# mobilinkd/m17-cxx-demod

Measured on AMD Instinct MI355X. Metric: Msamples/s demodulated (48 kSPS 4-FSK in -> decoded frames), higher is better.
Workload: dtype f32

## Files before the change

m17-cxx-demod_amd/csrc/m17_fir_skew_body.inc:

```
    __shared__ __attribute__((aligned(16))) float win[FS_LDS_FLOATS];
    const int tid = threadIdx.x;
    typedef int v4i __attribute__((ext_vector_type(4)));
    constexpr int NCH = (FS_WIN + 7) / 8;
    constexpr int CPT = (NCH + FS_THREADS - 1) / FS_THREADS;
    constexpr bool F32 = std::is_same<XT, float>::value;
    constexpr int FS_LAST = FS_WIN - 16 * FS_THREADS;
    static_assert(FS_LAST > 0 && FS_LAST <= FS_THREADS && CPT == 3, "the float form's split of the window");
    v4i pre[F32 ? 4 : CPT];
    int pre_last = 0;
    int m = 0;
    auto fetch = [&](uint32_t item) {
        const uint32_t c = item / tiles, tile = item - c * tiles;
        const XT* xr = x + (size_t)c * xpitch + XPRE;
        const int64_t w0 = (int64_t)tile * FS_TILE - FS_WOFF;
#pragma unroll
        for (int q = 0; q < CPT; ++q) {
            const int k = tid + q * FS_THREADS;
            const int64_t t = w0 + 8 * k;
            v4i v = {0, 0, 0, 0};
            if constexpr (F32) {
                if (q < 2) {
                    v4i v2 = {0, 0, 0, 0};
                    if (t + 8 <= (int64_t)T) {
                        v = *reinterpret_cast<const v4i*>(xr + t);
                        v2 = *reinterpret_cast<const v4i*>(xr + t + 4);
                    } else {
                        uint32_t w[8];
#pragma unroll
                        for (int h = 0; h < 8; ++h) w[h] = t + h < (int64_t)T ? __float_as_uint(xr[t + h]) : 0u;
                        v = v4i{(int)w[0], (int)w[1], (int)w[2], (int)w[3]};
                        v2 = v4i{(int)w[4], (int)w[5], (int)w[6], (int)w[7]};
                    }
                    pre[2 * q] = v; pre[2 * q + 1] = v2;
                } else {
                    const int64_t tl = w0 + 16 * FS_THREADS + tid;
                    pre_last = (tid < FS_LAST && tl < (int64_t)T) ? (int)__float_as_uint(xr[tl]) : 0;
                }
            } else {
            if (k < NCH) {
                if (t + 8 <= (int64_t)T) v = *reinterpret_cast<const v4i*>(xr + t);
                else {
                    uint32_t w[4] = {0u, 0u, 0u, 0u};
#pragma unroll 1
                    for (int h = 0; h < 8; ++h)
                        if (t + h < (int64_t)T) w[h >> 1] |= (uint32_t)(uint16_t)xr[t + h] << (16 * (h & 1));
                    v = v4i{(int)w[0], (int)w[1], (int)w[2], (int)w[3]};
                }
            }
            pre[q] = v;
            }
        }
    };
    auto stage = [&] {
#pragma unroll
        for (int q = 0; q < CPT; ++q) {
            const int k = tid + q * FS_THREADS;
            int sm = INVERT ? (int)0x80000000u : 0;
            if constexpr (F32 && MIXED) sm = m & (int)0x80000000u;
            if constexpr (F32) if (q == 2) {
                const int j = 16 * FS_THREADS + tid;
                if (tid < FS_LAST) win[FS_PADF + j + 2 * (j >> 4)] = __int_as_float(pre_last ^ sm);
                continue;
            }
            if (k < NCH) {
                float* dst = win + FS_PADF + 8 * k + 2 * (k >> 1);
                if constexpr (F32) {
#pragma unroll
                    for (int h = 0; h < 4; ++h) {
                        const v4i r = pre[2 * q + (h >> 1)];
                        const int a = ((h & 1) ? r[2] : r[0]) ^ sm, b = ((h & 1) ? r[3] : r[1]) ^ sm;
                        *reinterpret_cast<v2f*>(dst + 2 * h) = v2f{__int_as_float(a), __int_as_float(b)};
                    }
                } else
#pragma unroll
                for (int h = 0; h < 4; ++h) {
                    int w = pre[q][h];
// ... 80 lines not shown
```

m17-cxx-demod_amd/csrc/m17_frontend_kernels.hpp:

```cpp
#pragma once

#include "m17_common.hpp"

#include <type_traits>

namespace m17 {

typedef float v2f __attribute__((ext_vector_type(2)));

template <bool INVERT>
__device__ __forceinline__ v2f dcd_scale2(int a, int b)
{
    if (INVERT) { a = (int)(int16_t)(-a); b = (int)(int16_t)(-b); }
    const v2f rcp = {1.0f / 41067.0f, 1.0f / 41067.0f};
    const v2f k = {41067.0f, 41067.0f};
    const v2f fs = {(float)a, (float)b};
    const v2f q = fs * rcp;
    const v2f r = __builtin_elementwise_fma(-q, k, fs);
    return __builtin_elementwise_fma(r, rcp, q);
}

__device__ __forceinline__ int pol_mask(const uint32_t* __restrict__ pol, uint32_t c, uint32_t flip) { return -(int)((pol[c] ^ flip) & 1u); }
__device__ __forceinline__ int pol_word(int w, int m)
{
// ... 109 lines not shown
    }
}

#endif

template <int E, int N, typename F>
__device__ __forceinline__ void static_for(F&& f)
{
    if constexpr (E < N) {
        f(std::integral_constant<int, E>{});
        static_for<E + 1, N>(f);
    }
}

constexpr int FS_R = 16;
constexpr int FS_THREADS = 256;
constexpr int FS_TILE = FS_R * FS_THREADS;
constexpr int FS_WOFF = 152;
constexpr int FS_WIN = FS_TILE + FS_WOFF;
constexpr int FS_PADF = 18;
constexpr int FS_LDS_FLOATS = FS_PADF + ((FS_WIN + 15) / 16) * 18;
constexpr int FS_STEPS = 150, FS_BODY = 32, FS_ENTRY = 10, FS_NBODY = 5;
static_assert(FS_BODY - FS_ENTRY + (FS_NBODY - 1) * FS_BODY == FS_STEPS, "step count");
constexpr int FS_TAB = 64;

constexpr int fs_off(int e) { return e + 2 * ((e - (e < 0 ? 15 : 0)) / 16); }

inline void fs_build_tap_table(float* tab )
{
    auto T2 = [](int s) { return (s >= 1 && s <= 149) ? rrc_tap(s - 1) : 0.0f; };
    for (int bi = 0; bi < FS_NBODY; ++bi)
        for (int k = 0; k < 32; ++k) {
            const int s = 32 * (bi - 1) + (FS_BODY - FS_ENTRY) + k;
            tab[bi * FS_TAB + k] = T2(s);
            tab[bi * FS_TAB + 32 + k] = T2(s + 1);
        }
}

template <int HALF>
__device__ __forceinline__ v2f fs_tap_pair_times(v2f taps, v2f wpair)
{
    v2f r;
    if constexpr (HALF) asm("v_pk_mul_f32 %0, %1, %2 op_sel:[0,1] op_sel_hi:[1,1]" : "=v"(r) : "s"(taps), "v"(wpair));
    else asm("v_pk_mul_f32 %0, %1, %2 op_sel:[0,0] op_sel_hi:[1,0]" : "=v"(r) : "s"(taps), "v"(wpair));
    return r;
}

template <bool INVERT>
__global__ __launch_bounds__(FS_THREADS, 4) void fir_rrc150_skew_kernel(const int16_t* __restrict__ x, size_t xpitch, float* __restrict__ y, size_t ypitch,
                                                                       uint32_t T, const float* __restrict__ tab, uint32_t tiles, uint32_t items,
                                                                       const uint32_t* __restrict__ first_needed)
{
    constexpr bool MIXED = false;
    const uint32_t* pol = nullptr; const uint32_t flip = 0u;
    typedef int16_t XT;
#include "m17_fir_skew_body.inc"
}
__global__ __launch_bounds__(FS_THREADS, 4) void fir_rrc150_skew_mixed_kernel(const int16_t* __restrict__ x, size_t xpitch, float* __restrict__ y, size_t ypitch,
                                                                             uint32_t T, const float* __restrict__ tab, uint32_t tiles, uint32_t items,
                                                                             const uint32_t* __restrict__ first_needed, const uint32_t* __restrict__ pol, uint32_t flip)
{
    constexpr bool INVERT = false, MIXED = true;
    typedef int16_t XT;
#include "m17_fir_skew_body.inc"
}
template <bool INVERT>
__global__ __launch_bounds__(FS_THREADS, 4) void fir_rrc150_skew_f32_kernel(const float* __restrict__ x, size_t xpitch, float* __restrict__ y, size_t ypitch,
                                                                           uint32_t T, const float* __restrict__ tab, uint32_t tiles, uint32_t items,
                                                                           const uint32_t* __restrict__ first_needed)
{
    constexpr bool MIXED = false;
    const uint32_t* pol = nullptr; const uint32_t flip = 0u;
    typedef float XT;
#include "m17_fir_skew_body.inc"
}
__global__ __launch_bounds__(FS_THREADS, 4) void fir_rrc150_skew_mixed_f32_kernel(const float* __restrict__ x, size_t xpitch, float* __restrict__ y, size_t ypitch,
                                                                                 uint32_t T, const float* __restrict__ tab, uint32_t tiles, uint32_t items,
                                                                                 const uint32_t* __restrict__ first_needed, const uint32_t* __restrict__ pol, uint32_t flip)
{
    constexpr bool INVERT = false, MIXED = true;
    typedef float XT;
#include "m17_fir_skew_body.inc"
}

__global__ __launch_bounds__(256) void correlate_kernel(const float* __restrict__ y, size_t ypitch, float* __restrict__ corr,
                                                        uint32_t C, uint32_t T, uint32_t t0, uint32_t Ttot)
{
    const uint32_t c = blockIdx.y;
    const uint32_t t = t0 + blockIdx.x * blockDim.x + threadIdx.x;
    if (t >= t0 + T) return;
    const float* yr = y + (size_t)c * ypitch + YPRE;
// ... 461 lines not shown
```

m17-cxx-demod_amd/csrc/m17_gate_kernel.hpp:

```cpp
#pragma once

#include "m17_common.hpp"
#include "m17_decode_device.hpp"
#include "m17_frontend_kernels.hpp"
#include "m17_state.hpp"

namespace m17 {

struct GateExport {
    int32_t init;
    uint32_t on, trig, count;
    int32_t run_pos;
    float h0, h1, h2;
    float level;
    uint32_t seg;
    int32_t end_in_run, end_t;
};

struct GateParams {
    const int16_t* x;
    size_t xpitch;
    const float* y;
    size_t ypitch;
    float* h;
// ... 3 lines not shown
    const GateExport* chain_in;
    GateExport* chain_out;
    const uint32_t* only;
    const Boundary* bnd;
    float* final_h;
    const float* taps;
    uint32_t C, T;
    uint64_t pos0;
    uint64_t tick_row0;
    uint32_t flags;
    uint32_t nblk;
    EvParams ev;
    const uint32_t* pol;
    const float* hist_f;
    const float* bnd_hist_f;
};

constexpr int GT_LPC = 4;
constexpr int GT_CPW = 64 / GT_LPC;
constexpr int GT_ROW = TICK + 4;
constexpr int GT_F4 = TICK / 4 / GT_LPC;
constexpr int GT_LDS_FLOATS = GT_CPW * GT_ROW + GT_CPW * 148 + 298;

template <typename XT>
__device__ __forceinline__ void limit_track_pass(const GateParams& P, bool state_only, uint32_t c, bool valid, bool from_chain, const Boundary* bnd_base,
                                                 float* lds_base)
{
    constexpr uint32_t t0 = 0;
    const uint32_t segT = P.T;
    const size_t fh_off = 0;
    const Boundary* bnd = bnd_base ? bnd_base + c : nullptr;
    const uint64_t pos0 = P.pos0 + t0;
    float (&yl)[GT_CPW][GT_ROW] = *reinterpret_cast<float (*)[GT_CPW][GT_ROW]>(lds_base);
    float (&hl)[GT_CPW][GT_ROW] = yl;
    float (&pl)[GT_CPW][148] = *reinterpret_cast<float (*)[GT_CPW][148]>(lds_base + GT_CPW * GT_ROW);
    float (&pw)[298] = *reinterpret_cast<float (*)[298]>(lds_base + GT_CPW * GT_ROW + GT_CPW * 148);
    const int lane = threadIdx.x;
    const int g = lane % GT_CPW, r = lane / GT_CPW;
    const bool invert = ((P.flags ^ (P.pol ? P.pol[c] : 0u)) & 1u) != 0u;
    const bool store = !state_only;
    const SeqState* gs = P.state + c;
    const float* yr = P.y + (size_t)c * P.ypitch + YPRE + t0;
    float* hr = P.h + (size_t)c * P.ypitch + YPRE + t0;
    const float* tab = P.dcd_table + (size_t)c * P.ticks_cap * 12;

    int32_t init, run_pos, end_t = 0;
    uint32_t on, trig, count, seg;
    float h0, h1, h2, level;
    bool end_in_run = false;
    if (from_chain) {
        const GateExport e = P.chain_in[c];
// ... 8 lines not shown
        on = gs->hot.dcd_on; trig = gs->hot.dcd_trig; count = gs->hot.count;
        run_pos = gs->hot.run_pos;
        h0 = gs->hot.h0; h1 = gs->hot.h1; h2 = gs->hot.h2;
        level = gs->cold.dcd_level;
        seg = gs->cold.seg_start_tick;
    }
    if (!valid) { init = 0; on = 0; trig = 0; count = 0; run_pos = 148; h0 = h1 = h2 = 0.f; level = 0.f; seg = 0; end_in_run = false; end_t = 0; }
    if (!from_chain && r == 0 && valid && store) { hr[-1] = h0; hr[-2] = h1; hr[-3] = h2; }
    bool pl_valid = false;
    int32_t pl_rs = 0;

    auto lds_sync = [] {
        __builtin_amdgcn_fence(__ATOMIC_RELEASE, "wavefront", "local");
        __builtin_amdgcn_wave_barrier();
        __builtin_amdgcn_fence(__ATOMIC_ACQUIRE, "wavefront", "local");
    };
    auto dcd_update = [&](uint64_t k, float l1, float l2) {
        level = (float)((double)level * 0.8 + 0.2 * (double)(l1 / l2));
        seg = (uint32_t)(k + 1);
        trig = trig ? (level > 0.1f) : (level > 4.0f);
    };

    uint32_t t = 0;
    uint32_t phase = (uint32_t)(pos0 % TICK);
    uint64_t k_cur = pos0 / TICK;
    float4 pre[GT_F4];
#pragma unroll
    for (int b = 0; b < GT_F4; ++b) pre[b] = make_float4(0.f, 0.f, 0.f, 0.f);
    uint32_t pre_t = 0xFFFFFFFFu;
    auto stage_tick = [&]() {
// ... 92 lines not shown
                    const XT sv = eir ? xrc[(int64_t)et - 148 + k] : hist[k];
                    pw[k] = scale_sample(sv, inv_cc);
                }
                for (int k = lane; k < 148; k += 64)
                    if ((int64_t)rs + k < (int64_t)segT) pw[149 + k] = scale_sample(xrc[(int64_t)rs + k], inv_cc);
                lds_sync();
                for (int j = rp + lane; j < 148; j += 64) {
                    if ((int64_t)rs + j >= (int64_t)segT) break;
                    float acc = 0.f;
                    for (int i = 0; i < NTAPS; ++i) {
                        const float p = pw[149 + j - i] * P.taps[i];
                        acc = acc + p;
                    }
                    pl[gg][j] = acc;
                }
                lds_sync();
            }
            if (need_patch) { pl_valid = true; pl_rs = (int32_t)t - run_pos; }
        }
        const uint32_t te = t + n - 1u;
        const uint64_t k = k_cur;
        const uint64_t krow = min(k - P.tick_row0, (uint64_t)P.ticks_cap - 1);
        const float* row = tab + (size_t)krow * 12;
        const int jsum = (uint32_t)(k + 1 - seg) > 5 ? 5 : (int)(seg % 5u);
        const float l1 = row[jsum], l2 = row[6 + jsum];
        if (__ballot(feed)) {
            const bool overlay = feed && pl_valid && (int32_t)t - pl_rs < 148;
            const bool fast = n == TICK && ((pos0 + t) & 3u) == 0 && !__ballot(overlay);
            if (fast) {
                stage_tick();
            } else {
#pragma clang loop unroll(disable) vectorize(disable)
                for (uint32_t i = r; i < n; i += GT_LPC) {
                    float v = 0.f;
                    if (feed) {
                        const int32_t j = (int32_t)(t + i) - pl_rs;
                        v = (pl_valid && j < 148) ? pl[g][j] : yr[t + i];
                    }
                    yl[g][i] = v;
                }
            }
            lds_sync();
            if (r == 0 && feed) {
                if (n == TICK) {
                    iir_tick();
                } else {
                    float m2 = IirCoef::a2 * h1;
                    if ((n & 3u) == 0) {
#pragma clang loop unroll(disable)
                        for (uint32_t i = 0; i < n; i += 4) *reinterpret_cast<float4*>(&hl[g][i]) = four(*reinterpret_cast<const float4*>(&yl[g][i]), m2);
                    } else {
#pragma clang loop unroll(disable)
// ... 119 lines not shown
```

m17-cxx-demod_amd/csrc/m17hip.hip:

```cpp
#include "../../include/m17hip.h"

#include "m17_common.hpp"
#include "m17_decode_device.hpp"
#include "m17_frontend_kernels.hpp"
#include "m17_iq_kernels.hpp"
#include "m17_wide_kernels.hpp"
#include "m17_wide2_kernels.hpp"
#include "m17_state.hpp"
#include "m17_wave_kernel.hpp"
#include "m17_gate_kernel.hpp"
#include "m17_mod_kernels.hpp"
#include "m17_parity_kernels.hpp"
#include "m17_voice_kernel.hpp"
#include "m17_gather.hpp"

#include <hip/hip_ext.h>

#include <algorithm>
#include <cmath>
#include <complex>
#include <cstdio>
#include <cstdlib>
#include <cstring>
#include <ctime>
// ... 134 lines not shown
    int par_ = 0;
    Pass owed_; uint32_t pitch_ = 0, pitch_override_ = 0, maxC_ = 0;
    DevBuf<uint32_t> cur_;
};

struct TimedLaunch { Event a, b; int which; };

struct BertState; struct ChanStat; struct PacketState; struct PacketRec;

struct RunPlan {
    uint32_t C = 0, T = 0, flags = 0, nseg = 0;
    std::vector<uint32_t> b;
    bool staged = false, from_front = false;
    uint32_t ramp = 0;
    bool dcd_latency = false, fir_latency = false;
    bool gate_run = false;
    uint32_t front_segs = 0;
    bool gate0_queued = false;
    uint32_t n_reset = 0;
    uint32_t kflags = 0;
    const uint32_t* pol = nullptr;
    uint32_t t0(uint32_t k) const { return b[std::min<size_t>(k, nseg)]; }
};

}

struct m17hip_ctx {
    int device = 0;
    int last_hip = 0;
    hipStream_t stream = nullptr;
// ... 64 lines not shown
    bool stage_inputs = false;
    DevBuf<char> synth_scratch;
    uint32_t runT = 0;
    Event ev_tail;
    int gate0_early = 1;
    DevBuf<Boundary> bnd;
    uint32_t front_k1_after = 0;
    uint32_t last_nseg = 0;
    bool wave_times = false;
    uint32_t stagedC = 0, stagedT = 0;
    bool front_queued = false;
    RunPlan front_plan;
    uint32_t carryT = 0;
    DevBuf<float> final_h;
    DevBuf<GateExport> gate_exp;
    DevBuf<uint32_t> dropped;
    DevBuf<BertState> bert_state;
    bool bert = false;
    DevBuf<ChanStat> chan_words;
    DevBuf<PacketState> pkt_state;
    DevBuf<PacketRec> pkt_recs2[2];
    DevBuf<uint32_t> pkt_count2;
    uint32_t pkt_cap = 0;
    bool pkt_fed = false;
    DevBuf<VoiceState> voice_state;
    DevBuf<uint8_t> voice_audio2[2];
    DevBuf<uint8_t> voice_marks2[2];
    DevBuf<uint32_t> voice_counts2;
    DevBuf<CallRec> call_recs2[2];
    DevBuf<uint32_t> call_counts2;
// ... 37 lines not shown
    Event ev_switch;
    Event ev_fetch;
    DevBuf<uint32_t> overflow;
    DevBuf<uint64_t> rec_offsets;
    DevBuf<FrameRec> compact;
    DevBuf<DecodeTables> tables;
    DevBuf<float> taps;
    DevBuf<float> taps_skew;
    int limit_form = 1;
    int fir_form = 1;
    int gate_aware = -1;
    DevBuf<GateTruth> truth;
    DevBuf<uint32_t> first_needed;
    uint32_t off_segs_prev = 0, chan_segs_prev = 0;
    uint32_t fir_grid = 0;
    uint32_t n_cu = 256;
    DevBuf<uint32_t> defer_hist;
    bool defer_decode = true;
    bool defer_evm = true;
    EvmFold evm;
    uint32_t seq_lds_bytes = 0;
    DevBuf<float> llr_edges;
    DevBuf<core::Kalman2Gain> level_gain;
    DevBuf<char> scratch;
    DcdCoef coef{};
    uint64_t pos = 0;
    std::vector<uint32_t> marks;
    std::vector<uint8_t> marked;
    TurnTable reset_list;
    std::vector<uint8_t> pol_host;
// ... 533 lines not shown
    uint64_t run = partial[tid];
    for (uint32_t c = lo; c < hi; ++c) { offsets[c] = run; run += min(counts[c], rec_cap); }
}

__global__ void compact_kernel(const FrameRec* recs, uint32_t rec_cap, const uint32_t* counts, const uint64_t* offsets,
                               FrameRec* out, uint64_t out_cap, uint32_t C)
{
    const uint32_t c = blockIdx.x;
    const uint32_t n = min(counts[c], rec_cap);
    const uint4* src = reinterpret_cast<const uint4*>(recs + (size_t)c * rec_cap);
    uint4* dst = reinterpret_cast<uint4*>(out + offsets[c]);
    for (uint32_t k = threadIdx.x; k < n * 4; k += blockDim.x)
        if (offsets[c] + k / 4 < out_cap) dst[k] = src[k];
}

constexpr size_t SEQ_LDS_BYTES_4 = 34816;
constexpr uint32_t FIR_GRID_PER_CU = 5, FIR_ITEMS_LATENCY = 3, FIR_ITEMS_THROUGHPUT = 8;
int launch_fir(m17hip_ctx* c, uint32_t C, uint32_t T, uint32_t flags, bool latency, hipStream_t st, uint32_t t0 = 0, const uint32_t* first_needed = nullptr,
               const uint32_t* pol = nullptr)
{
    TimedK tm(c, KT_FIR);
#ifdef M17_TOOLS
    if (c->fir_form == 0 && c->f32_now()) return M17HIP_ESTATE;
    if (c->fir_form == 0 && pol) return M17HIP_EINVAL;
    if (c->fir_form == 0) {
        dim3 grid((T + FIR_TILE - 1) / FIR_TILE, C);
        tm.launch((fir_rrc150_rolled_kernel<FIR_R, 4>), grid, dim3(FIR_THREADS), 0, st, c->now().x + t0, c->xpitch, c->now().y + t0, c->ypitch, T, flags, c->taps);
    } else
#endif
    {
        const uint32_t tiles = (T + FS_TILE - 1) / FS_TILE;
        const uint64_t items64 = (uint64_t)tiles * C;
        if (items64 > 0xFFFFFFFFull) return M17HIP_EINVAL;
        const uint32_t items = (uint32_t)items64;
        const uint32_t per = latency ? FIR_ITEMS_LATENCY : FIR_ITEMS_THROUGHPUT;
        const uint32_t cap = c->fir_grid ? c->fir_grid : std::max(FIR_GRID_PER_CU * c->n_cu, (items + per - 1) / per);
        const dim3 grid(std::min(items, cap));
        const auto go = [&](auto kernel, const auto* xin, auto... mixed) {
            tm.launch(kernel, grid, dim3(FS_THREADS), 0, st, xin + t0, c->xpitch, c->now().y + t0, c->ypitch, T, c->taps_skew, tiles, items, first_needed, mixed...);
        };
        if (c->f32_now()) {
            const float* xf = c->fslab[c->slot].x;
            if (pol) go(fir_rrc150_skew_mixed_f32_kernel, xf, pol, flags & 1u);
            else if (flags & 1u) go(fir_rrc150_skew_f32_kernel<true>, xf);
            else go(fir_rrc150_skew_f32_kernel<false>, xf);
        } else {
            const int16_t* xi = c->now().x;
            if (pol) go(fir_rrc150_skew_mixed_kernel, xi, pol, flags & 1u);
            else if (flags & 1u) go(fir_rrc150_skew_kernel<true>, xi);
            else go(fir_rrc150_skew_kernel<false>, xi);
        }
    }
    HIPCHK(c, hipGetLastError());
    return M17HIP_OK;
}
int launch_dcd(m17hip_ctx* c, uint32_t C, uint32_t T, uint32_t flags, uint64_t pos, bool latency, hipStream_t st, uint32_t t0 = 0, const uint32_t* pol = nullptr)
{
    TimedK tm(c, KT_DCD);
    const uint64_t row0 = (pos + t0) / TICK - pos / TICK;
    const bool one_wave = !latency || T % DP_BLK != 0 || (pos + t0) % DP_BLK != 0 || t0 % 8 != 0 || T < 4 * DP_BLK;
    const dim3 grid(one_wave ? (C + DCD_CPW * DCD_WPB - 1) / (DCD_CPW * DCD_WPB) : (C + DP_CPB - 1) / DP_CPB), block(one_wave ? 64 * DCD_WPB : 256);
    const auto go = [&](auto kernel, const auto* xin, auto... mixed) {
        tm.launch(kernel, grid, block, 0, st, xin + t0, c->xpitch, c->dcd_state, c->now().dcd + row0 * 12, c->ticks_cap, C, T, pos + t0, c->coef, flags, mixed...);
    };
    if (c->f32_now()) {
// ... 102 lines not shown
    c->xpitch = round_up((size_t)XPRE + max_samples + 8, 8);
    c->ypitch = round_up((size_t)YPRE + max_samples + 4, 4);
    static_assert(M17HIP_MAX_SAMPLES_PER_RUN == (0x7FFF0000u / (4u * GT_CPW)) - 256u, "include/m17hip.h: M17HIP_MAX_SAMPLES_PER_RUN");
    if ((size_t)GT_CPW * c->ypitch * 4u > (size_t)0x7FFF0000u) return fail(M17HIP_EINVAL);
    c->ticks_cap = max_samples / TICK + 2;
    c->rec_cap = c->rec_cap_alloc = 2 * (max_samples / 1920 + 2) + 4;
    const size_t C = max_channels;
    int r = M17HIP_OK;
    auto alloc = [&](auto& buf, size_t n) { if (!r) r = alloc_code(c, buf.alloc(n)); };
    m17hip_ctx::Slab& s = c->slab[0];
    alloc(s.x, C * c->xpitch);
    alloc(s.y, C * c->ypitch);
    alloc(s.h, C * c->ypitch);
    alloc(c->final_h, 2 * C * 4);
    alloc(c->gate_exp, C);
    alloc(c->dropped, 2 * C);
    alloc(c->bert_state, C);
    alloc(s.dcd, C * c->ticks_cap * 12);
    alloc(c->dcd_state, C);
    alloc(c->seq_state, C);
    alloc(c->evm.state, C);
    alloc(c->evm, C);
    alloc(c->sets[0].recs, C * c->rec_cap);
    alloc(c->sets[0].rec_count, C);
    alloc(c->rec_offsets, C + 1);
    alloc(c->overflow, 8);
    alloc(c->tables, 1);
    alloc(c->taps, 160);
    alloc(c->taps_skew, FS_NBODY * FS_TAB);
    alloc(c->llr_edges, 64);
// ... 743 lines not shown
    hipLaunchKernelGGL(mod_shape_kernel, dim3((T + 255) / 256, C), dim3(256), 0, in.st, mp, C, T, chan0, sym, sym_pitch, nsym, in.x, c->xpitch);
    HIPCHK(c, hipGetLastError());
    HIPCHK(c, hipStreamSynchronize(in.st));
    input_done(c, in, C, T);
    return M17HIP_OK;
}

int m17hip_fir_rrc150(m17hip_ctx* c, uint32_t C, uint32_t T, uint32_t flags, float* out_host)
{
    if (!c || C == 0 || T == 0 || C > c->maxC || T > c->maxT || (flags & ~M17HIP_FLAG_INVERT)) return M17HIP_EINVAL;
    GUARD(c);
    if (c->front_queued) return M17HIP_ESTATE;
    if (!c->uploaded) return M17HIP_ESTATE;
    uint32_t kflags; const uint32_t* pol;
    if (int r = resolve_polarity(c, C, flags, c->stream, kflags, pol)) return r;
    if (int r = launch_fir(c, C, T, kflags, false, c->stream, 0, nullptr, pol)) return r;
    if (out_host) {
        HIPCHK(c, hipMemcpy2DAsync(out_host, (size_t)T * sizeof(float), c->now().y + YPRE, c->ypitch * sizeof(float), (size_t)T * sizeof(float), C,
                                   hipMemcpyDeviceToHost, c->stream));
    }
    HIPCHK(c, hipStreamSynchronize(c->stream));
    return M17HIP_OK;
}

int m17hip_correlator(m17hip_ctx* c, uint32_t C, uint32_t T, float* limit_host, float* corr_host)
{
    if (!c || C == 0 || T == 0 || C > c->maxC || T > c->maxT) return M17HIP_EINVAL;
    GUARD(c);
    if (c->front_queued) return M17HIP_ESTATE;
    const size_t n = (size_t)C * T;
    HIPCHK(c, c->scratch.grow(5 * n * sizeof(float), &c->last_hip));
// ... 254 lines not shown
}

enum RunKind { RUN_IN_PLACE, RUN_STAGED, RUN_STAGED_FRONT };
static RunPlan plan_run(m17hip_ctx* c, uint32_t C, uint32_t T, uint32_t flags, RunKind kind)
{
    RunPlan p;
    p.C = C; p.T = T; p.flags = p.kflags = flags; p.staged = kind != RUN_IN_PLACE; p.from_front = kind == RUN_STAGED_FRONT;
    const bool ask = kind == RUN_IN_PLACE || (kind == RUN_STAGED && c->dcd_form < 0);
    const bool chain_bound = !ask || !runs_overlap(c);
    p.ramp = c->seg_ramp > 0 ? (uint32_t)c->seg_ramp : (c->seg_ramp < 0 && kind == RUN_IN_PLACE && chain_bound) ? AUTO_RAMP : 0u;
    p.b = segment_bounds(c, T, p.ramp); p.nseg = (uint32_t)p.b.size() - 1u;
    p.front_segs = std::min(c->front_ahead ? c->front_ahead : p.nseg, p.nseg);
    const bool want = c->gate_aware == 1 || (c->gate_aware < 0 && c->chan_segs_prev && 4ull * c->off_segs_prev > (uint64_t)c->chan_segs_prev);
    p.gate_run = want && p.nseg >= 3u && !c->front_ahead && !c->profile;
    p.fir_latency = c->dcd_form < 0 ? chain_bound : c->dcd_form == 1;
    p.dcd_latency = p.fir_latency || (p.gate_run && c->dcd_form < 0);
    return p;
}

static int launch_front_seg(m17hip_ctx* c, const RunPlan& p, uint32_t k)
{
    if (k >= p.nseg) return M17HIP_OK;
    auto& seg = c->now().seg;
    const uint32_t ahead = p.front_segs, t0 = p.t0(k), len = p.t0(k + 1) - t0;
    if (k >= ahead) {
        HIPCHK(c, hipStreamWaitEvent(c->side, seg[k - ahead].seq, 0));
        HIPCHK(c, hipStreamWaitEvent(c->side2, seg[k - ahead].seq, 0));
    }
    if (k == 1) HIPCHK(c, hipStreamWaitEvent(c->side, seg[0].fir, 0));
    if (int r = launch_dcd(c, p.C, len, p.kflags, c->pos, p.dcd_latency, c->side, t0, p.pol)) return r;
    HIPCHK(c, hipEventRecord(seg[k].dcd, c->side));
    if (p.gate_run && k >= 2u) return M17HIP_OK;
    if (int r = launch_fir(c, p.C, len, p.kflags, p.fir_latency, c->side2, t0, nullptr, p.pol)) return r;
    HIPCHK(c, hipEventRecord(seg[k].fir, c->side2));
    return M17HIP_OK;
}

static int launch_front_all(m17hip_ctx* c, const RunPlan& p)
{
    HIPCHK(c, c->now().ensure_seg_events(p.nseg));
    if (!p.staged) {
        HIPCHK(c, hipEventRecord(c->ev_fork, c->stream));
        HIPCHK(c, hipStreamWaitEvent(c->side, c->ev_fork, 0));
        HIPCHK(c, hipStreamWaitEvent(c->side2, c->ev_fork, 0));
    }
    for (uint32_t k = 0; k < p.front_segs; ++k)
        if (int r = launch_front_seg(c, p, k)) return r;
    return M17HIP_OK;
}

static int launch_gated_fir(m17hip_ctx* c, const RunPlan& p, uint32_t k)
{
    if (k + 2u >= p.nseg) return M17HIP_OK;
    auto& seg = c->now().seg;
    const uint32_t C = p.C, t1 = p.t0(k + 1u), t2 = p.t0(k + 2u), t3 = p.t0(k + 3u);
    HIPCHK(c, hipStreamWaitEvent(c->side2, seg[k].seq, 0));
    HIPCHK(c, hipStreamWaitEvent(c->side2, seg[k + 2u].dcd, 0));
    hipLaunchKernelGGL(gate_forecast_kernel, dim3((C + 63) / 64), dim3(64), 0, c->side2, by_parity(c->truth, k, c->maxC), c->now().dcd, c->ticks_cap,
                       (uint64_t)(c->pos / TICK), (uint64_t)(c->pos + t1), t2 - t1, t3 - t1, c->first_needed, C);
    HIPCHK(c, hipGetLastError());
    if (int r = launch_fir(c, C, t3 - t2, p.kflags, p.fir_latency, c->side2, t2, c->first_needed, p.pol)) return r;
    HIPCHK(c, hipEventRecord(seg[k + 2u].fir, c->side2));
    return M17HIP_OK;
}

static EvParams ev_fold(const m17hip_ctx* c, const EvmFold::Pass& f, EvLast last) { return EvParams{f.ops, c->evm.pitch(), c->evm.state, c->diag_cap ? c->diag_log : nullptr, c->diag_cap, c->seq_state, f.C, f.upto, last}; }
static EvParams ev_no_fold(uint32_t C) { return EvParams{nullptr, 0, nullptr, nullptr, 0, nullptr, C, nullptr, 0u}; }

static int launch_gate_seg(m17hip_ctx* c, const RunPlan& p, uint32_t k, hipStream_t st, bool ahead, bool redo, bool redo_stores = false)
{
    if (k == 0 && p.gate0_queued) {
        HIPCHK(c, hipStreamWaitEvent(st, c->now().seg[0].gate, 0));
        return M17HIP_OK;
    }
    const uint32_t C = p.C, t0 = p.t0(k), len = p.t0(k + 1) - t0;
    TimedK tm(c, KT_GATE);
    GateParams G{};
    G.x = c->x_now(t0); G.xpitch = c->xpitch; G.y = c->now().y + t0; G.ypitch = c->ypitch; G.h = c->now().h + t0;
    G.dcd_table = c->now().dcd; G.ticks_cap = c->ticks_cap; G.state = c->seq_state;
    G.final_h = by_parity(c->final_h, k, c->maxC, 4);
    G.chain_in = ahead ? c->gate_exp : nullptr; G.chain_out = c->gate_exp;
    G.only = redo ? by_parity(c->dropped, k - 1u, c->maxC) : nullptr;
    G.bnd = redo ? by_parity(c->bnd, k, c->maxC) : nullptr;
    const bool f32 = c->f32_now();
    if (f32) { G.hist_f = c->hist_f; G.bnd_hist_f = redo ? by_parity(c->bnd_hist_f, k, c->maxC, HISTF_PITCH) : nullptr; }
    G.taps = c->taps; G.C = C; G.T = len; G.pos0 = c->pos + t0; G.tick_row0 = c->pos / TICK; G.flags = p.kflags | ((redo && !redo_stores) ? 2u : 0u); G.pol = p.pol;
    G.nblk = (C + GT_CPW - 1) / GT_CPW;
    uint32_t fold_blocks = 0;
    if (ahead && k >= 2 && c->defer_evm && c->evm.ops()) {
        G.ev = ev_fold(c, c->evm.ahead(k, C), EV_MORE);
        fold_blocks = ev_fold_blocks(C);
    }
    if (!redo && c->evm.owed() && ((p.nseg >= 2 && ahead && k == 1) || (p.nseg < 2 && k == 0))) {
        const EvmFold::Pass f = c->evm.take();
        G.ev = ev_fold(c, f, k == 0 ? EV_SETTLES : EV_BESIDE_K5);
        fold_blocks = f.blocks();
    }
    if (f32) tm.launch(limit_track_f32_kernel, dim3(G.nblk + fold_blocks), dim3(64), GT_LDS_FLOATS * sizeof(float), st, G);
    else tm.launch(limit_track_kernel, dim3(G.nblk + fold_blocks), dim3(64), GT_LDS_FLOATS * sizeof(float), st, G);
    HIPCHK(c, hipGetLastError());
    return M17HIP_OK;
}
// ... 177 lines not shown
    uint32_t npieces = (T + piece - 1) / piece;
    if (tiled && npieces > 1 && T - (npieces - 1) * piece < 4 * LP_TILE) --npieces;
    HIPCHK(c, c->now().ensure_seg_events(npieces));
    int r;
    uint32_t kflags; const uint32_t* pol;
    if ((r = resolve_polarity(c, C, flags, c->stream, kflags, pol))) return r;
    auto& seg = c->now().seg;
    const hipStream_t st_chain = c->stream, st_fir = c->side2, st_corr = c->side;
    const uint32_t chain_wgs = (C + LP_CH - 1) / LP_CH;
    HIPCHK(c, hipEventRecord(c->ev_fork, c->stream));
    for (hipStream_t st : {st_chain, st_fir, st_corr})
        if (st != c->stream) HIPCHK(c, hipStreamWaitEvent(st, c->ev_fork, 0));
    if (tiled) HIPCHK(c, hipMemsetAsync(lstate, 0, (size_t)C * 4 * sizeof(float), st_chain));
    for (uint32_t k = 0; k < npieces; ++k) {
        const uint32_t t0 = k * piece, len = k + 1 < npieces ? piece : T - t0;
        if ((r = launch_fir(c, C, len, kflags, false, st_fir, t0, nullptr, pol))) return r;
        HIPCHK(c, hipEventRecord(seg[k].fir, st_fir));
        HIPCHK(c, hipStreamWaitEvent(st_corr, seg[k].fir, 0));
        HIPCHK(c, hipStreamWaitEvent(st_chain, seg[k].fir, 0));
        {
            Timed tc(c, KT_CORR, st_corr);
            if (T % 4 == 0 && t0 % 4 == 0 && len % 4 == 0)
                hipLaunchKernelGGL(correlate4_kernel, dim3((len / 4 + 255) / 256, C), dim3(256), 0, st_corr, c->now().y, c->ypitch, corr, C, len, t0, T);
            else
                hipLaunchKernelGGL(correlate_kernel, dim3((len + 255) / 256, C), dim3(256), 0, st_corr, c->now().y, c->ypitch, corr, C, len, t0, T);
        }
        Timed tm(c, KT_GATE, st_chain);
#ifdef M17_TOOLS
        if (tiled && c->limit_form == 0)
            hipLaunchKernelGGL(limit_pipe_kernel, dim3(chain_wgs), dim3(320), 0, st_chain, c->now().y + t0, c->ypitch, limit + t0, (size_t)T, C, len,
                               (const float*)lstate, lstate);
// ... 1011 lines not shown
    case 31:
        if (value < 0 || value > 0x7FFFFFFF) return M17HIP_EINVAL;
        c->gather_timeout_ms = (uint32_t)value;
        return M17HIP_OK;
    case 16:
        c->stage_inputs = value != 0;
        return M17HIP_OK;
    case 26:
        if (value < -1 || value > 1) return M17HIP_EINVAL;
        c->gate_aware = (int)value;
        return M17HIP_OK;
    case 33:
        if (value < -1 || value > 0x7FFFFFFF) return M17HIP_EINVAL;
        c->seg_ramp = value;
        return M17HIP_OK;
    case 13:
        if (value < 0 || value > (1 << 20)) return M17HIP_EINVAL;
        c->fir_grid = (uint32_t)value;
        return M17HIP_OK;
#ifdef M17_TOOLS
    case 27:
        if (value < 0 || value > 1) return M17HIP_EINVAL;
        c->limit_form = (int)value;
        return M17HIP_OK;
    case 11:
        if (value < 0 || value > 1) return M17HIP_EINVAL;
        c->fir_form = (int)value;
        return M17HIP_OK;
    case 1:
        c->profile = value != 0;
// ... 80 lines not shown
```

Baseline: 102,000.

## Move gate patch buffer to global memory and add optional two-wave FIR

Moves the gate kernel's per-column 148-float patch rows out of LDS into a device buffer, and trims the sequencer's LDS reservation. Together these let four K5 workgroups, a gate workgroup and a FIR workgroup share one CU's LDS. It also templates the skewed FIR kernels on thread count and adds an option for a 128-thread variant with smaller tiles and a larger grid. The patch reads now go through global memory instead of LDS, which may cost latency on the slow path.

After: 99170. 0.972x the previous value.

```diff
diff --git a/m17-cxx-demod_amd/csrc/m17_fir_skew_body.inc b/m17-cxx-demod_amd/csrc/m17_fir_skew_body.inc
--- a/m17-cxx-demod_amd/csrc/m17_fir_skew_body.inc
+++ b/m17-cxx-demod_amd/csrc/m17_fir_skew_body.inc
@@ -1,3 +1,4 @@
+    constexpr int FS_THREADS = NT, FS_TILE = fs_tile(NT), FS_WIN = fs_win(NT), FS_LDS_FLOATS = fs_lds_floats(NT);
     __shared__ __attribute__((aligned(16))) float win[FS_LDS_FLOATS];
     const int tid = threadIdx.x;
     typedef int v4i __attribute__((ext_vector_type(4)));
@@ -5,9 +6,10 @@
     constexpr int CPT = (NCH + FS_THREADS - 1) / FS_THREADS;
     constexpr bool F32 = std::is_same<XT, float>::value;
     constexpr int FS_LAST = FS_WIN - 16 * FS_THREADS;
-    static_assert(FS_LAST > 0 && FS_LAST <= FS_THREADS && CPT == 3, "the float form's split of the window");
+    constexpr int LPT = (FS_LAST + FS_THREADS - 1) / FS_THREADS;
+    static_assert(FS_LAST > 0 && LPT <= 2 && CPT == 3, "the float form's split of the window");
     v4i pre[F32 ? 4 : CPT];
-    int pre_last = 0;
+    int pre_last = 0, pre_last2 = 0;
     int m = 0;
     auto fetch = [&](uint32_t item) {
         const uint32_t c = item / tiles, tile = item - c * tiles;
@@ -26,8 +28,10 @@
                         v2 = *reinterpret_cast<const v4i*>(xr + t + 4);
                     } else {
                         uint32_t w[8];
+                        int64_t tr = t;
+                        if constexpr (NT != 256) asm volatile("" : "+v"(tr));
 #pragma unroll
-                        for (int h = 0; h < 8; ++h) w[h] = t + h < (int64_t)T ? __float_as_uint(xr[t + h]) : 0u;
+                        for (int h = 0; h < 8; ++h) w[h] = tr + h < (int64_t)T ? __float_as_uint(xr[tr + h]) : 0u;
                         v = v4i{(int)w[0], (int)w[1], (int)w[2], (int)w[3]};
                         v2 = v4i{(int)w[4], (int)w[5], (int)w[6], (int)w[7]};
                     }
@@ -35,6 +39,7 @@
                 } else {
                     const int64_t tl = w0 + 16 * FS_THREADS + tid;
                     pre_last = (tid < FS_LAST && tl < (int64_t)T) ? (int)__float_as_uint(xr[tl]) : 0;
+                    if constexpr (LPT > 1) pre_last2 = (tid + FS_THREADS < FS_LAST && tl + FS_THREADS < (int64_t)T) ? (int)__float_as_uint(xr[tl + FS_THREADS]) : 0;
                 }
             } else {
             if (k < NCH) {
@@ -60,6 +65,10 @@
             if constexpr (F32) if (q == 2) {
                 const int j = 16 * FS_THREADS + tid;
                 if (tid < FS_LAST) win[FS_PADF + j + 2 * (j >> 4)] = __int_as_float(pre_last ^ sm);
+                if constexpr (LPT > 1) {
+                    const int j2 = j + FS_THREADS;
+                    if (tid + FS_THREADS < FS_LAST) win[FS_PADF + j2 + 2 * (j2 >> 4)] = __int_as_float(pre_last2 ^ sm);
+                }
                 continue;
             }
             if (k < NCH) {
diff --git a/m17-cxx-demod_amd/csrc/m17_frontend_kernels.hpp b/m17-cxx-demod_amd/csrc/m17_frontend_kernels.hpp
--- a/m17-cxx-demod_amd/csrc/m17_frontend_kernels.hpp
+++ b/m17-cxx-demod_amd/csrc/m17_frontend_kernels.hpp
@@ -147,12 +147,12 @@
 }
 
 constexpr int FS_R = 16;
-constexpr int FS_THREADS = 256;
-constexpr int FS_TILE = FS_R * FS_THREADS;
 constexpr int FS_WOFF = 152;
-constexpr int FS_WIN = FS_TILE + FS_WOFF;
 constexpr int FS_PADF = 18;
-constexpr int FS_LDS_FLOATS = FS_PADF + ((FS_WIN + 15) / 16) * 18;
+constexpr int fs_tile(int nt) { return FS_R * nt; }
+constexpr int fs_win(int nt) { return fs_tile(nt) + FS_WOFF; }
+constexpr int fs_lds_floats(int nt) { return FS_PADF + ((fs_win(nt) + 15) / 16) * 18; }
+static_assert(fs_lds_floats(256) * 4 == 19224 && fs_lds_floats(128) * 4 == 10008, "K1's LDS per workgroup (m17hip.hip: the CU's LDS budget)");
 constexpr int FS_STEPS = 150, FS_BODY = 32, FS_ENTRY = 10, FS_NBODY = 5;
 static_assert(FS_BODY - FS_ENTRY + (FS_NBODY - 1) * FS_BODY == FS_STEPS, "step count");
 constexpr int FS_TAB = 64;
@@ -179,8 +179,8 @@
     return r;
 }
 
-template <bool INVERT>
-__global__ __launch_bounds__(FS_THREADS, 4) void fir_rrc150_skew_kernel(const int16_t* __restrict__ x, size_t xpitch, float* __restrict__ y, size_t ypitch,
+template <bool INVERT, int NT>
+__global__ __launch_bounds__(NT, 4) void fir_rrc150_skew_kernel(const int16_t* __restrict__ x, size_t xpitch, float* __restrict__ y, size_t ypitch,
                                                                        uint32_t T, const float* __restrict__ tab, uint32_t tiles, uint32_t items,
                                                                        const uint32_t* __restrict__ first_needed)
 {
@@ -189,7 +189,8 @@
     typedef int16_t XT;
 #include "m17_fir_skew_body.inc"
 }
-__global__ __launch_bounds__(FS_THREADS, 4) void fir_rrc150_skew_mixed_kernel(const int16_t* __restrict__ x, size_t xpitch, float* __restrict__ y, size_t ypitch,
+template <int NT>
+__global__ __launch_bounds__(NT, 4) void fir_rrc150_skew_mixed_kernel(const int16_t* __restrict__ x, size_t xpitch, float* __restrict__ y, size_t ypitch,
                                                                              uint32_t T, const float* __restrict__ tab, uint32_t tiles, uint32_t items,
                                                                              const uint32_t* __restrict__ first_needed, const uint32_t* __restrict__ pol, uint32_t flip)
 {
@@ -197,8 +198,8 @@
     typedef int16_t XT;
 #include "m17_fir_skew_body.inc"
 }
-template <bool INVERT>
-__global__ __launch_bounds__(FS_THREADS, 4) void fir_rrc150_skew_f32_kernel(const float* __restrict__ x, size_t xpitch, float* __restrict__ y, size_t ypitch,
+template <bool INVERT, int NT>
+__global__ __launch_bounds__(NT, 4) void fir_rrc150_skew_f32_kernel(const float* __restrict__ x, size_t xpitch, float* __restrict__ y, size_t ypitch,
                                                                            uint32_t T, const float* __restrict__ tab, uint32_t tiles, uint32_t items,
                                                                            const uint32_t* __restrict__ first_needed)
 {
@@ -207,7 +208,8 @@
     typedef float XT;
 #include "m17_fir_skew_body.inc"
 }
-__global__ __launch_bounds__(FS_THREADS, 4) void fir_rrc150_skew_mixed_f32_kernel(const float* __restrict__ x, size_t xpitch, float* __restrict__ y, size_t ypitch,
+template <int NT>
+__global__ __launch_bounds__(NT, 4) void fir_rrc150_skew_mixed_f32_kernel(const float* __restrict__ x, size_t xpitch, float* __restrict__ y, size_t ypitch,
                                                                                  uint32_t T, const float* __restrict__ tab, uint32_t tiles, uint32_t items,
                                                                                  const uint32_t* __restrict__ first_needed, const uint32_t* __restrict__ pol, uint32_t flip)
 {
diff --git a/m17-cxx-demod_amd/csrc/m17_gate_kernel.hpp b/m17-cxx-demod_amd/csrc/m17_gate_kernel.hpp
--- a/m17-cxx-demod_amd/csrc/m17_gate_kernel.hpp
+++ b/m17-cxx-demod_amd/csrc/m17_gate_kernel.hpp
@@ -41,13 +41,16 @@
     const uint32_t* pol;
     const float* hist_f;
     const float* bnd_hist_f;
+    float* patch;
 };
 
 constexpr int GT_LPC = 4;
 constexpr int GT_CPW = 64 / GT_LPC;
 constexpr int GT_ROW = TICK + 4;
 constexpr int GT_F4 = TICK / 4 / GT_LPC;
-constexpr int GT_LDS_FLOATS = GT_CPW * GT_ROW + GT_CPW * 148 + 298;
+constexpr int GT_LDS_FLOATS = GT_CPW * GT_ROW + 298;
+constexpr int GT_PATCH_FLOATS = 148;
+static_assert(GT_LDS_FLOATS * 4 >= 4352, "the EVM fold pass's LDS");
 
 template <typename XT>
 __device__ __forceinline__ void limit_track_pass(const GateParams& P, bool state_only, uint32_t c, bool valid, bool from_chain, const Boundary* bnd_base,
@@ -60,8 +63,8 @@
     const uint64_t pos0 = P.pos0 + t0;
     float (&yl)[GT_CPW][GT_ROW] = *reinterpret_cast<float (*)[GT_CPW][GT_ROW]>(lds_base);
     float (&hl)[GT_CPW][GT_ROW] = yl;
-    float (&pl)[GT_CPW][148] = *reinterpret_cast<float (*)[GT_CPW][148]>(lds_base + GT_CPW * GT_ROW);
-    float (&pw)[298] = *reinterpret_cast<float (*)[298]>(lds_base + GT_CPW * GT_ROW + GT_CPW * 148);
+    float (*pl)[148] = reinterpret_cast<float (*)[148]>(P.patch) + (size_t)blockIdx.x * GT_CPW;
+    float (&pw)[298] = *reinterpret_cast<float (*)[298]>(lds_base + GT_CPW * GT_ROW);
     const int lane = threadIdx.x;
     const int g = lane % GT_CPW, r = lane / GT_CPW;
     const bool invert = ((P.flags ^ (P.pol ? P.pol[c] : 0u)) & 1u) != 0u;
@@ -100,6 +103,11 @@
         __builtin_amdgcn_fence(__ATOMIC_RELEASE, "wavefront", "local");
         __builtin_amdgcn_wave_barrier();
         __builtin_amdgcn_fence(__ATOMIC_ACQUIRE, "wavefront", "local");
+    };
+    auto patch_sync = [] {
+        __builtin_amdgcn_fence(__ATOMIC_RELEASE, "wavefront");
+        __builtin_amdgcn_wave_barrier();
+        __builtin_amdgcn_fence(__ATOMIC_ACQUIRE, "wavefront");
     };
     auto dcd_update = [&](uint64_t k, float l1, float l2) {
         level = (float)((double)level * 0.8 + 0.2 * (double)(l1 / l2));
@@ -222,7 +230,7 @@
                     }
                     pl[gg][j] = acc;
                 }
-                lds_sync();
+                patch_sync();
             }
             if (need_patch) { pl_valid = true; pl_rs = (int32_t)t - run_pos; }
         }
@@ -238,12 +246,15 @@
             if (fast) {
                 stage_tick();
             } else {
+                uint32_t prow = (uint32_t)g;
+                asm volatile("" : "+v"(prow));
+                const float* plg = pl[prow];
 #pragma clang loop unroll(disable) vectorize(disable)
                 for (uint32_t i = r; i < n; i += GT_LPC) {
                     float v = 0.f;
                     if (feed) {
                         const int32_t j = (int32_t)(t + i) - pl_rs;
-                        v = (pl_valid && j < 148) ? pl[g][j] : yr[t + i];
+                        v = (pl_valid && j < 148) ? plg[j] : yr[t + i];
                     }
                     yl[g][i] = v;
                 }
diff --git a/m17-cxx-demod_amd/csrc/m17hip.hip b/m17-cxx-demod_amd/csrc/m17hip.hip
--- a/m17-cxx-demod_amd/csrc/m17hip.hip
+++ b/m17-cxx-demod_amd/csrc/m17hip.hip
@@ -172,6 +172,7 @@
     bool staged = false, from_front = false;
     uint32_t ramp = 0;
     bool dcd_latency = false, fir_latency = false;
+    bool fir_two_wave = false;
     bool gate_run = false;
     uint32_t front_segs = 0;
     bool gate0_queued = false;
@@ -266,6 +267,8 @@
     uint32_t carryT = 0;
     DevBuf<float> final_h;
     DevBuf<GateExport> gate_exp;
+    DevBuf<float> gate_patch;
+    size_t patch_rows = 0;
     DevBuf<uint32_t> dropped;
     DevBuf<BertState> bert_state;
     bool bert = false;
@@ -333,6 +336,7 @@
     DevBuf<uint32_t> first_needed;
     uint32_t off_segs_prev = 0, chan_segs_prev = 0;
     uint32_t fir_grid = 0;
+    int fir_threads = -1;
     uint32_t n_cu = 256;
     DevBuf<uint32_t> defer_hist;
     bool defer_decode = true;
@@ -896,9 +900,14 @@
         if (offsets[c] + k / 4 < out_cap) dst[k] = src[k];
 }
 
-constexpr size_t SEQ_LDS_BYTES_4 = 34816;
+constexpr size_t LDS_PER_CU = 163840, LDS_GRANULE = 1280;
+constexpr size_t lds_granules(size_t bytes) { return (bytes + LDS_GRANULE - 1) / LDS_GRANULE; }
+constexpr size_t SEQ_LDS_BYTES_4 = 33280;
+static_assert(SEQ_LDS_BYTES_4 * 5 > LDS_PER_CU && SEQ_LDS_BYTES_4 >= (size_t)wave_lds_words(4) * 4, "K5: four workgroups per CU, not five; at least its need");
+static_assert(4 * lds_granules(SEQ_LDS_BYTES_4) + lds_granules(GT_LDS_FLOATS * 4) + lds_granules(fs_lds_floats(128) * 4) <= LDS_PER_CU / LDS_GRANULE,
+              "four K5 workgroups, a K2 workgroup and a two-wave K1 workgroup share a CU");
 constexpr uint32_t FIR_GRID_PER_CU = 5, FIR_ITEMS_LATENCY = 3, FIR_ITEMS_THROUGHPUT = 8;
-int launch_fir(m17hip_ctx* c, uint32_t C, uint32_t T, uint32_t flags, bool latency, hipStream_t st, uint32_t t0 = 0, const uint32_t* first_needed = nullptr,
+int launch_fir(m17hip_ctx* c, uint32_t C, uint32_t T, uint32_t flags, bool latency, bool two_wave, hipStream_t st, uint32_t t0 = 0, const uint32_t* first_needed = nullptr,
                const uint32_t* pol = nullptr)
 {
     TimedK tm(c, KT_FIR);
@@ -911,26 +920,40 @@
     } else
 #endif
     {
-        const uint32_t tiles = (T + FS_TILE - 1) / FS_TILE;
+        const bool w2 = two_wave;
+        const uint32_t tile = w2 ? fs_tile(128) : fs_tile(256);
+        const uint32_t tiles = (T + tile - 1) / tile;
         const uint64_t items64 = (uint64_t)tiles * C;
         if (items64 > 0xFFFFFFFFull) return M17HIP_EINVAL;
         const uint32_t items = (uint32_t)items64;
-        const uint32_t per = latency ? FIR_ITEMS_LATENCY : FIR_ITEMS_THROUGHPUT;
-        const uint32_t cap = c->fir_grid ? c->fir_grid : std::max(FIR_GRID_PER_CU * c->n_cu, (items + per - 1) / per);
+        const uint32_t per = (latency ? FIR_ITEMS_LATENCY : FIR_ITEMS_THROUGHPUT) * (w2 ? 2u : 1u);
+        const uint32_t cap = c->fir_grid ? c->fir_grid : std::max(FIR_GRID_PER_CU * (w2 ? 2u : 1u) * c->n_cu, (items + per - 1) / per);
         const dim3 grid(std::min(items, cap));
         const auto go = [&](auto kernel, const auto* xin, auto... mixed) {
-            tm.launch(kernel, grid, dim3(FS_THREADS), 0, st, xin + t0, c->xpitch, c->now().y + t0, c->ypitch, T, c->taps_skew, tiles, items, first_needed, mixed...);
+            tm.launch(kernel, grid, dim3(w2 ? 128 : 256), 0, st, xin + t0, c->xpitch, c->now().y + t0, c->ypitch, T, c->taps_skew, tiles, items, first_needed, mixed...);
         };
         if (c->f32_now()) {
             const float* xf = c->fslab[c->slot].x;
-            if (pol) go(fir_rrc150_skew_mixed_f32_kernel, xf, pol, flags & 1u);
-            else if (flags & 1u) go(fir_rrc150_skew_f32_kernel<true>, xf);
-            else go(fir_rrc150_skew_f32_kernel<false>, xf);
+            if (w2) {
+                if (pol) go(fir_rrc150_skew_mixed_f32_kernel<128>, xf, pol, flags & 1u);
+                else if (flags & 1u) go((fir_rrc150_skew_f32_kernel<true, 128>), xf);
+                else go((fir_rrc150_skew_f32_kernel<false, 128>), xf);
+            } else {
+                if (pol) go(fir_rrc150_skew_mixed_f32_kernel<256>, xf, pol, flags & 1u);
+                else if (flags & 1u) go((fir_rrc150_skew_f32_kernel<true, 256>), xf);
+                else go((fir_rrc150_skew_f32_kernel<false, 256>), xf);
+            }
         } else {
             const int16_t* xi = c->now().x;
-            if (pol) go(fir_rrc150_skew_mixed_kernel, xi, pol, flags & 1u);
-            else if (flags & 1u) go(fir_rrc150_skew_kernel<true>, xi);
-            else go(fir_rrc150_skew_kernel<false>, xi);
+            if (w2) {
+                if (pol) go(fir_rrc150_skew_mixed_kernel<128>, xi, pol, flags & 1u);
+                else if (flags & 1u) go((fir_rrc150_skew_kernel<true, 128>), xi);
+                else go((fir_rrc150_skew_kernel<false, 128>), xi);
+            } else {
+                if (pol) go(fir_rrc150_skew_mixed_kernel<256>, xi, pol, flags & 1u);
+                else if (flags & 1u) go((fir_rrc150_skew_kernel<true, 256>), xi);
+                else go((fir_rrc150_skew_kernel<false, 256>), xi);
+            }
         }
     }
     HIPCHK(c, hipGetLastError());
@@ -1063,6 +1086,8 @@
     alloc(s.h, C * c->ypitch);
     alloc(c->final_h, 2 * C * 4);
     alloc(c->gate_exp, C);
+    c->patch_rows = round_up(C, (size_t)GT_CPW);
+    alloc(c->gate_patch, 4 * c->patch_rows * GT_PATCH_FLOATS);
     alloc(c->dropped, 2 * C);
     alloc(c->bert_state, C);
     alloc(s.dcd, C * c->ticks_cap * 12);
@@ -1836,7 +1861,7 @@
     if (!c->uploaded) return M17HIP_ESTATE;
     uint32_t kflags; const uint32_t* pol;
     if (int r = resolve_polarity(c, C, flags, c->stream, kflags, pol)) return r;
-    if (int r = launch_fir(c, C, T, kflags, false, c->stream, 0, nullptr, pol)) return r;
+    if (int r = launch_fir(c, C, T, kflags, false, c->fir_threads == 128, c->stream, 0, nullptr, pol)) return r;
     if (out_host) {
         HIPCHK(c, hipMemcpy2DAsync(out_host, (size_t)T * sizeof(float), c->now().y + YPRE, c->ypitch * sizeof(float), (size_t)T * sizeof(float), C,
                                    hipMemcpyDeviceToHost, c->stream));
@@ -2121,6 +2146,7 @@
     const bool want = c->gate_aware == 1 || (c->gate_aware < 0 && c->chan_segs_prev && 4ull * c->off_segs_prev > (uint64_t)c->chan_segs_prev);
     p.gate_run = want && p.nseg >= 3u && !c->front_ahead && !c->profile;
     p.fir_latency = c->dcd_form < 0 ? chain_bound : c->dcd_form == 1;
+    p.fir_two_wave = c->fir_threads == 128;
     p.dcd_latency = p.fir_latency || (p.gate_run && c->dcd_form < 0);
     return p;
 }
@@ -2138,7 +2164,7 @@
     if (int r = launch_dcd(c, p.C, len, p.kflags, c->pos, p.dcd_latency, c->side, t0, p.pol)) return r;
     HIPCHK(c, hipEventRecord(seg[k].dcd, c->side));
     if (p.gate_run && k >= 2u) return M17HIP_OK;
-    if (int r = launch_fir(c, p.C, len, p.kflags, p.fir_latency, c->side2, t0, nullptr, p.pol)) return r;
+    if (int r = launch_fir(c, p.C, len, p.kflags, p.fir_latency, p.fir_two_wave, c->side2, t0, nullptr, p.pol)) return r;
     HIPCHK(c, hipEventRecord(seg[k].fir, c->side2));
     return M17HIP_OK;
 }
@@ -2166,7 +2192,7 @@
     hipLaunchKernelGGL(gate_forecast_kernel, dim3((C + 63) / 64), dim3(64), 0, c->side2, by_parity(c->truth, k, c->maxC), c->now().dcd, c->ticks_cap,
                        (uint64_t)(c->pos / TICK), (uint64_t)(c->pos + t1), t2 - t1, t3 - t1, c->first_needed, C);
     HIPCHK(c, hipGetLastError());
-    if (int r = launch_fir(c, C, t3 - t2, p.kflags, p.fir_latency, c->side2, t2, c->first_needed, p.pol)) return r;
+    if (int r = launch_fir(c, C, t3 - t2, p.kflags, p.fir_latency, p.fir_two_wave, c->side2, t2, c->first_needed, p.pol)) return r;
     HIPCHK(c, hipEventRecord(seg[k + 2u].fir, c->side2));
     return M17HIP_OK;
 }
@@ -2193,6 +2219,7 @@
     if (f32) { G.hist_f = c->hist_f; G.bnd_hist_f = redo ? by_parity(c->bnd_hist_f, k, c->maxC, HISTF_PITCH) : nullptr; }
     G.taps = c->taps; G.C = C; G.T = len; G.pos0 = c->pos + t0; G.tick_row0 = c->pos / TICK; G.flags = p.kflags | ((redo && !redo_stores) ? 2u : 0u); G.pol = p.pol;
     G.nblk = (C + GT_CPW - 1) / GT_CPW;
+    G.patch = c->gate_patch + (size_t)(2 * c->slot + (redo ? 1 : 0)) * c->patch_rows * GT_PATCH_FLOATS;
     uint32_t fold_blocks = 0;
     if (ahead && k >= 2 && c->defer_evm && c->evm.ops()) {
         G.ev = ev_fold(c, c->evm.ahead(k, C), EV_MORE);
@@ -2400,7 +2427,7 @@
     if (tiled) HIPCHK(c, hipMemsetAsync(lstate, 0, (size_t)C * 4 * sizeof(float), st_chain));
     for (uint32_t k = 0; k < npieces; ++k) {
         const uint32_t t0 = k * piece, len = k + 1 < npieces ? piece : T - t0;
-        if ((r = launch_fir(c, C, len, kflags, false, st_fir, t0, nullptr, pol))) return r;
+        if ((r = launch_fir(c, C, len, kflags, false, c->fir_threads == 128, st_fir, t0, nullptr, pol))) return r;
         HIPCHK(c, hipEventRecord(seg[k].fir, st_fir));
         HIPCHK(c, hipStreamWaitEvent(st_corr, seg[k].fir, 0));
         HIPCHK(c, hipStreamWaitEvent(st_chain, seg[k].fir, 0));
@@ -3442,6 +3469,10 @@
         if (value < -1 || value > 0x7FFFFFFF) return M17HIP_EINVAL;
         c->seg_ramp = value;
         return M17HIP_OK;
+    case 35:
+        if (value != -1 && value != 256 && value != 128) return M17HIP_EINVAL;
+        c->fir_threads = (int)value;
+        return M17HIP_OK;
     case 13:
         if (value < 0 || value > (1 << 20)) return M17HIP_EINVAL;
         c->fir_grid = (uint32_t)value;
```
